# fukangl/SMG-multimodal-grasping

Hardware: AMD Instinct MI355X
Metric: affordance fwd+bwd passes/sec (16-rot 224^2 RGB-D) (higher is better)
Workload: dtype f32; 1 GPU; 16 rot x 224^2 (S=640): fwd + Huber + bwd + Adam per GPU per step; reinforcement_net style 0; 17 trunk passes; fp32; leg=headline, rotations=16, input_size=640, parallelism=dp1

## Files before the change

### smg-multimodal-grasping_amd/csrc/backward.hip

```cpp
#include "engine.h"

int do_backward(smg_engine* e, const smg_net* net, const float* dq, hipStream_t st, int phases, bool elem_head) {
    if (!e->have_fwd) return fail(-22, "smg_backward without a preceding smg_forward");
    if (!net->grads) return fail(-22, "net.grads is NULL");
    if (phases == 2 && !e->bw_phase0_done)
        return fail(-22, "smg_backward_phase(1) must follow smg_backward_phase(0) of the same forward");
    if ((phases & 1) && e->bw_phase0_done)
        return fail(-22, "smg_backward / smg_backward_phase(0) while the second half of a two-phase backward is still due (run phase 1 or a new forward)");
    const Layout& L = *e->L;
    const TrunkRef& T = L.trunk[e->f_trunk];
    const HeadRef& Hd = L.head[e->f_head];
    const int NS = e->f_streams, NP = e->f_pairs;
    const float* P = net->params;
    float* Gr = net->grads;
    const Plane p4 = e->p_blk[3];
    const bool ph_a = phases & 1, ph_b = phases & 2;
    if (ph_a) {
        for (int r = 0; r < kStatRep; ++r) HIP_OK(hipMemsetAsync(e->bstat + (size_t)r * kStatRepStride, 0, 2 * e->bstat_span * sizeof(double), st));
    }
    const bool split16 = e->prec == 0 && kSplitOp == 3;
    if (ph_a && split16) HIP_OK(hipMemsetAsync(e->gamax, 0, (size_t)e->gamax_words * sizeof(unsigned), st));
    const hipStream_t s2 = (e->prof || e->serialize) ? st : e->side;
    auto fork = [&](hipEvent_t ev) -> int {
        HIP_OK(hipEventRecord(ev, st));
        HIP_OK(hipStreamWaitEvent(s2, ev, 0));
        return 0;
    };
    const bool gs_materialised = split16 || NS > 4;
    auto gs_on_side = [&](const Plane& pl) { return split16 && !e->generic3x3 && pl.HW <= 1600 && NS <= 4; };
    auto fused_gsrc = [&](int b, const DenseLayerRef& d) {
        return grad_src(e, e->G[b], kBlockCtot[b], e->X[b], kBlockCtot[b], e->st_X[b], d.cin, nullptr);
    };
    auto launch_gs_apply = [&](int b, int i, hipStream_t cs, float* GSb, const GradSrc& fused) {
        const Plane pl = e->p_blk[b];
        BnBwdApplyArgs a{};
        a.src = fused; a.src.xtab = stat_table(e, e->sx_tab[b], e->max_streams, kBlockCtot[b], T.layers[b][i].cin);
        a.pl = pl; a.C = kGrowth;
        a.out = GSb; a.ldo = kGrowth; a.amax = split16 ? gamax_of(e, b, i, 0) : nullptr;
        PREC_DISPATCH(e, launch_kernel(e, bn_bwd_apply_kernel<PREC>, dim3((pl.HWp + bn_apply_rows(PREC) - 1) / bn_apply_rows(PREC), NS), dim3(256), 0, cs,
                                       K_OTHER, 0, ESZ(e) * NS * pl.HW * 3 * kGrowth, false, a));
    };

    auto norm1_src = [&](int b, int i, int c0) {
        const DenseLayerRef& d = T.layers[b][i];
        return act_src(e, e->X[b], kBlockCtot[b], e->st_X[b], c0, P + d.n1.w, P + d.n1.b, stat_table(e, e->sx_tab[b], e->max_streams, kBlockCtot[b]), asc_n1(e, b, i));
    };
    auto norm2_src = [&](int b, int i) {
        const DenseLayerRef& d = T.layers[b][i];
        return act_src(e, el(e, e->Bt, e->bt_off[b][i]), kBottleneck, e->st_Bt[b][i], 0, P + d.n2.w, P + d.n2.b,
                       !e->generic3x3 ? stat_table(e, e->sb_tab[b][i], e->max_streams, kBottleneck) : StatTab{}, asc_n2(e, b, i));
    };

    PartialTiles tiles(e->part_floats, NS, e->deterministic);

    if (ph_a) {
    {
        ValueBwdArgs a;
        a.h1 = head_norm1_src(e, Hd, P); a.p4 = p4; a.w2p = e->packed_f + e->pk_head1;
        a.dq = dq; a.out_ch = e->head_out; a.OH = e->OH; a.OW = e->OW; a.dh1 = e->DH1;
        a.st = stat_sink_bwd(e, e->st_H1, 0); a.aff = affine_sink(Gr, Hd.n1); a.dw2 = Gr + Hd.c1.w;
        const bool dense = !elem_head && (e->head_bwd == 2 || (e->head_bwd == 0 && e->f_dense_dq));
        if (!dense) {
// ... 190 lines not shown
                a.wu = e->packed_u + e->pk_hd[b][i];
                const double flops = 2.0 * NS * pl.HW * 9 * kBottleneck * kGrowth;
                const double bytes = ESZ(e) * NS * pl.HW * (kGrowth + 2 * kBottleneck);
                if (halo_tile(pl, NS) == 16) {
                    a.tiles_x = (pl.W + 15) / 16; a.cg_per_wg = kBottleneck / 32;
                    if (pl.H % 16 || pl.W % 16) {
                        PREC_DISPATCH(e, launch_kernel(e, conv3x3_halo_dgrad_kernel<16, PREC, true>, dim3(((pl.H + 15) / 16) * a.tiles_x, NS), dim3(256),
                                                       HaloDgradSGeo<16, PREC>::smem_bytes(kBottleneck), st, K_D3, flops, bytes, true, a));
                    } else {
                        PREC_DISPATCH(e, launch_kernel(e, conv3x3_halo_dgrad_kernel<16, PREC>, dim3((pl.H / 16) * a.tiles_x, NS), dim3(256),
                                                       HaloDgradSGeo<16, PREC>::smem_bytes(kBottleneck), st, K_D3, flops, bytes, true, a));
                    }
                } else {
                    a.tiles_x = (pl.W + 7) / 8; a.cg_per_wg = 1;
                    PREC_DISPATCH(e, launch_kernel(e, conv3x3_halo_dgrad_kernel<8, PREC>, dim3(((pl.H + 7) / 8) * a.tiles_x, NS, kBottleneck / 64), dim3(256),
                                                   HaloDgradSGeo<8, PREC>::smem_bytes(kBottleneck), st, K_D3, flops, bytes, true, a));
                }
            } else {
                auto run = [&](auto tag) {
                    using Cfg = decltype(tag);
                    BwdDataP<Cfg, true, E_STORE, false> p{};
                    p.gs = grad_done(GSb, kGrowth); p.pa = pl; p.KA = kGrowth;
                    p.wp = e->packed_u + e->pk_g3d[b][i]; p.K8tot = 9 * kGrowth / 8; p.ldn = kBottleneck; p.wcol0 = 0; p.N = kBottleneck;
                    p.m = n2; p.pm = pl;
                    p.dst = split16 ? e->DY2 : D2b; p.ldd = kBottleneck; p.dcoff = 0;
                    p.st = n2st; p.aff = affine_sink(Gr, d.n2);
                    launch_gemm(e, st, p, dim3(NS * pl.HWp / Cfg::BM, kBottleneck / Cfg::BN), K_D3, 2.0 * NS * pl.HW * 9 * kBottleneck * kGrowth,
                                ESZ(e) * NS * pl.HW * (kGrowth + 2 * kBottleneck));
                };
                if (pl.HWp % 128 == 0) run(CfgP128x128{}); else run(CfgP64x128{});
            }
            const GradSrc dy2 = grad_src(e, split16 ? e->DY2 : D2b, kBottleneck, bt, kBottleneck, e->st_Bt[b][i], 0, P + d.n2.w,
                                         !e->generic3x3 ? stat_table(e, e->sb_tab[b][i], e->max_streams, kBottleneck) : StatTab{});
            if (split16) {
                BnBwdApplySplitArgs a{};
                a.src = dy2; a.pl = pl; a.out = reinterpret_cast<u32x4*>(D2b); a.binv = lb.D2S;
                if (!e->generic3x3) a.aff = affine_sink(Gr, d.n2);
                launch_kernel(e, bn_bwd_apply_split_kernel, dim3(pl.HWp / kScaleBlock, NS), dim3(256), 0, st, K_OTHER, 0, 4.0 * NS * pl.HW * 3 * kBottleneck, false, a);
            } else {
                if (e->dbg_stop == b * 100 + i) {
                    if (int rc = dbg_snapshot(e->dbg_dy2, e->dbg_dy2_floats, e->dbg_dy2_n, D2b, (int64_t)NS * pl.HWp * kBottleneck)) return rc;
                }
                BnBwdApplyArgs a{};
                a.src = dy2; a.pl = pl; a.C = kBottleneck; a.out = D2b; a.ldo = kBottleneck;
                if (!e->generic3x3) a.aff = affine_sink(Gr, d.n2);
                PREC_DISPATCH(e, launch_kernel(e, bn_bwd_apply_kernel<PREC>, dim3((pl.HWp + bn_apply_rows(PREC) - 1) / bn_apply_rows(PREC), NS), dim3(256), 0, st,
                                               K_OTHER, 0, ESZ(e) * NS * pl.HW * 3 * kBottleneck, false, a));
            }
            if (fork(e->ev_d2[lb.ring % kRing])) return -5;
            if (int rc = issue_wgrads(b, i)) return rc;
            HIP_OK(hipEventRecord(e->ev_side[lb.ring % kRing], s2));
            if (e->dbg_stop == b * 100 + i) {
                if (int rc = dbg_snapshot(e->dbg_gsnap, e->dbg_gsnap_floats, e->dbg_gsnap_n, e->G[b], (int64_t)NS * pl.HWp * Ct)) return rc;
            }
            const int L = (int)T.layers[b].size();
            const int g_lo = i - ((L - 1 - i) % kGroup == kGroup - 1 ? 0 : std::min(i, kGroup - 1 - (L - 1 - i) % kGroup));
            const int cs = T.layers[b][g_lo].cin;
            if (d.cin > cs) {
                auto run = [&](auto tag, auto ptag) {
                    using Cfg = MC<decltype(tag), decltype(ptag)::value>;
                    BwdDataP<Cfg, false, E_ACCUM, false, decltype(ptag)::value> p{};
                    p.gs = grad_done(D2b, kBottleneck); p.pa = pl; p.KA = kBottleneck; p.binv = lb.D2S;
                    p.wp = e->packed_u + e->pk_d1[b][i]; p.K8tot = kBottleneck / 8; p.ldn = d.cin; p.wcol0 = cs; p.N = d.cin - cs;
                    p.m = norm1_src(b, i, cs); p.pm = pl;
                    p.dst = e->G[b]; p.ldd = Ct; p.dcoff = cs;
                    p.st = stat_sink_bwd(e, e->st_X[b], cs); p.aff = affine_sink_scr(e, e->db_off[b][i], d.cin, cs);
                    launch_gemm(e, st, p, dim3(NS * pl.HWp / Cfg::BM, (p.N + Cfg::BN - 1) / Cfg::BN), K_D1, 2.0 * NS * pl.HW * p.N * kBottleneck,
                                ESZ(e) * NS * pl.HW * (kBottleneck + 3.0 * p.N));
                };
                PREC_DISPATCH(e, if (pl.HWp % 128 == 0) run(CfgP128x64{}, PTAG); else run(CfgP64x64{}, PTAG));
            }
            if (i == g_lo) {
                auto run = [&](auto tag, auto ptag) {
                    using Cfg = MC<decltype(tag), decltype(ptag)::value>;
                    BwdDataGroupP<Cfg, decltype(ptag)::value> p{};
                    const int g_hi = L - 1 - ((L - 1 - g_lo) / kGroup) * kGroup;
                    p.nseg = g_hi - g_lo + 1;
                    for (int k = 0; k < p.nseg; ++k) {
                        const DenseLayerRef& dk = T.layers[b][g_lo + k];
                        const LayerBuf lk = buf_of(b, g_lo + k);
                        p.seg[k].g = lk.D2; p.seg[k].wp = e->packed_u + e->pk_d1[b][g_lo + k]; p.seg[k].ldn = dk.cin; p.seg[k].binv = lk.D2S;
                        p.seg[k].gamma = P + dk.n1.w; p.seg[k].beta = P + dk.n1.b;
                        p.seg[k].aff = affine_sink_scr(e, e->db_off[b][g_lo + k], dk.cin, 0);
                    }
                    p.ldg = kBottleneck; p.pa = pl; p.KA = kBottleneck; p.N = cs;
                    p.m = act_src(e, e->X[b], Ct, e->st_X[b], 0, nullptr, nullptr, stat_table(e, e->sx_tab[b], e->max_streams, Ct));
                    p.dst = e->G[b]; p.ldd = Ct;
                    p.st = stat_sink_bwd(e, e->st_X[b], 0);
                    launch_gemm(e, st, p, dim3(NS * pl.HWp / Cfg::BM, (cs + Cfg::BN - 1) / Cfg::BN), K_D1, 2.0 * NS * pl.HW * cs * kBottleneck * p.nseg,
                                ESZ(e) * NS * pl.HW * ((double)p.nseg * kBottleneck + 3.0 * cs));
                };
// ... 125 lines not shown
```

### smg-multimodal-grasping_amd/csrc/elem.cuh

```cuda
#pragma once
#include "gemm.cuh"

namespace smg {

struct PrepArgs {
    const float* images_nchw;
    const double* heightmaps;
    int hm, pad, S;
    double mean, stdv;
    const int* stream_image;
    const float* stream_affine;
    const int* stream_rotated;
    float* img4;
    float* img1;
    int HWp;
    const double* masks;
    const int* stream_mask_a;
    const int* stream_mask_b;
};

__device__ __forceinline__ float lin_coord(int i, int S, float step) {
    return (i < S / 2) ? fmaf(step, (float)i, -1.f) : fmaf(-step, (float)(S - 1 - i), 1.f);
}

// ... 1089 lines not shown
            if constexpr (E == 4) {
                const float4 o = affine2(gv[k], xv[k], prm + 4 * cs, a.C);
                stq<GT>(a.out, pix * a.ldo + 4 * cs, o);
                vmax = fmaxf(fmaxf(vmax, fmaxf(fabsf(o.x), fabsf(o.y))), fmaxf(fabsf(o.z), fabsf(o.w)));
            } else {
                const u32x4 u = pack_unit<1>(affine2(slot_quad<GT>(gv[k], 0), slot_quad<XT>(xv[k], 0), prm + 8 * cs, a.C),
                                             affine2(slot_quad<GT>(gv[k], 1), slot_quad<XT>(xv[k], 1), prm + 8 * cs + 4, a.C));
                *reinterpret_cast<u32x4*>(static_cast<char*>(a.out) + (int64_t)GT::size * (pix * a.ldo + 8 * cs)) = u;
            }
        }
    }
    if constexpr (E == 4) {
        if (a.amax) {
#pragma unroll
            for (int o = 32; o > 0; o >>= 1) vmax = fmaxf(vmax, __shfl_xor(vmax, o));
            __syncthreads();
            if ((t & 63) == 0) prm[t >> 6] = vmax;
            __syncthreads();
            if (t == 0) {
                vmax = fmaxf(fmaxf(prm[0], prm[1]), fmaxf(prm[2], prm[3]));
                if (vmax > 0.f) atomicMax(a.amax + (int64_t)n * kAmaxRep + (blockIdx.x % kAmaxRep), __float_as_uint(vmax));
            }
        }
    }
}

struct BnBwdApplySplitArgs {
    GradSrc src;
    Plane pl;
    u32x4* out;
    float* binv;
    AffineSink aff;
};
static __global__ __launch_bounds__(256) void bn_bwd_apply_split_kernel(const BnBwdApplySplitArgs a) {
    constexpr int C = 8 * kD2K8;
    __shared__ float prm[4 * C];
    __shared__ float red[4];
    const int n = blockIdx.y, t = threadIdx.x;
    const int cs = t >> 3, rr = t & 7;
    const int r0 = blockIdx.x * kScaleBlock + rr;
    float4 gv[8], xv[8];
#pragma unroll
    for (int k = 0; k < 8; ++k) {
        const int r = r0 + 8 * k;
        const int64_t pix = (int64_t)n * a.pl.HWp + (r < a.pl.HW ? r : 0);
        gv[k] = ld4(static_cast<const float*>(a.src.g) + pix * C + 4 * cs);
        xv[k] = ld4(static_cast<const float*>(a.src.x) + pix * C + 4 * cs);
    }
    if (t < C) {
        const double inv = 1.0 / (double)a.pl.HW;
        float mean, invstd;
        const GradSrc& g = a.src;
        tab_or_moments(g.xtab, n, t, g.xsum, g.xsq, (int64_t)n * g.sstride + t, inv, g.eps, mean, invstd);
        const double s1 = stat_get(g.s1, (int64_t)n * g.sstride + t), s2 = stat_get(g.s2, (int64_t)n * g.sstride + t);
        prm[t] = g.gamma[t] * invstd;
        prm[C + t] = (float)(s1 * inv);
        prm[2 * C + t] = mean;
        prm[3 * C + t] = invstd * (float)(s2 * inv);
        if (a.aff.dbeta && blockIdx.x == 0) affine_sink_add2(a.aff, t, (float)s1, (float)s2);
    }
    __syncthreads();
    float vmax = 0.f;
#pragma unroll
    for (int k = 0; k < 8; ++k) {
        const float4 o = r0 + 8 * k < a.pl.HW ? affine2(gv[k], xv[k], prm + 4 * cs, C) : zero4();
        gv[k] = o;
        vmax = fmaxf(fmaxf(vmax, fmaxf(fabsf(o.x), fabsf(o.y))), fmaxf(fabsf(o.z), fabsf(o.w)));
    }
#pragma unroll
    for (int o = 32; o > 0; o >>= 1) vmax = fmaxf(vmax, __shfl_xor(vmax, o));
    if ((t & 63) == 0) red[t >> 6] = vmax;
    __syncthreads();
    vmax = fmaxf(fmaxf(red[0], red[1]), fmaxf(red[2], red[3]));
    ActScale sc{1.f, 1.f};
    if (vmax > 0.f) sc = scale_of_max(__float_as_uint(vmax));
    if (t == 0) a.binv[(int64_t)n * (a.pl.HWp / kScaleBlock) + blockIdx.x] = sc.inv;
    char* ob = reinterpret_cast<char*>(a.out + d2_stream_units(n, a.pl.HWp));
#pragma unroll
    for (int k = 0; k < 8; ++k) {
        const Split4 s = split4<3>(mul4(gv[k], sc.s));
        const int64_t at = ((int64_t)(cs >> 1) * a.pl.HWp + r0 + 8 * k) * 16 + (cs & 1) * 8;
        *reinterpret_cast<uint2*>(ob + at) = s.p[0];
        *reinterpret_cast<uint2*>(ob + at + (int64_t)kD2K8 * a.pl.HWp * 16) = s.p[1];
    }
}

struct DbSegD { int64_t grad_off; int scr_off; int n; };
static __global__ void db_flush_kernel(const DbSegD* segs, float* scr, int rep_stride, int reps, float* grads,
                                       const double* stem1, const double* stem2, int ns, float* dbeta0, float* dgamma0) {
    if (blockIdx.y == gridDim.y - 1) {
        if (blockIdx.x == 0 && threadIdx.x < 128 && stem1) {
            const int q = threadIdx.x >> 6, c = threadIdx.x & 63;
            double v = 0.0;
            for (int n = 0; n < ns; ++n) v += stat_get(q ? stem2 : stem1, (int64_t)n * 64 + c);
            (q ? dgamma0 : dbeta0)[c] += (float)v;
        }
        return;
    }
    const DbSegD sg = segs[blockIdx.y];
    for (int k = blockIdx.x * blockDim.x + threadIdx.x; k < sg.n; k += gridDim.x * blockDim.x) {
        float v = 0.f;
        for (int r = 0; r < reps; ++r) {
            float* q = scr + (int64_t)r * rep_stride + sg.scr_off + k;
            v += *q;
            *q = 0.f;
        }
        grads[sg.grad_off + k] += v;
    }
}

template <int PREC>
static __global__ void zero_uncovered_kernel(void* G, int ld, Plane p, int Hc, int Wc, int C) {
    using GT = grd_t<PREC>;
    const int n = blockIdx.y;
    const int64_t total = (int64_t)p.HW * (C / 4);
    for (int64_t i = blockIdx.x * (int64_t)blockDim.x + threadIdx.x; i < total; i += (int64_t)gridDim.x * blockDim.x) {
        const int pix = (int)(i / (C / 4)), cq = (int)(i - (int64_t)pix * (C / 4));
// ... 219 lines not shown
```

### smg-multimodal-grasping_amd/csrc/engine.h

```cpp
#pragma once
#include <hip/hip_runtime.h>

#include <algorithm>
#include <cmath>
#include <cstdio>
#include <cstdlib>
#include <cstring>
#include <string>
#include <type_traits>
#include <vector>

#include "../../include/smg_hip.h"
#include "elem.cuh"
#include "scene.cuh"
#include "gemm.cuh"
#include "halo.cuh"
#include "ws.cuh"
#include "wsw.cuh"
#include "plan.h"

using namespace smg;

int smg_fail(int code, const std::string& msg);
static inline int fail(int code, const std::string& msg) { return smg_fail(code, msg); }
#define HIP_OK(expr)                                                                              \
    do {                                                                                          \
        hipError_t _e = (expr);                                                                   \
        if (_e != hipSuccess)                                                                     \
            return fail(-5, std::string(#expr) + ": " + hipGetErrorString(_e));                   \
    } while (0)

static const Layout& layout_for(int head_out) {
    static Layout L1 = build_layout(1);
    static Layout L3 = build_layout(3);
    return head_out == 3 ? L3 : L1;
}

using CfgP128x128 = GemmCfg<128, 128, 16, 2, 2, 1, true>;
using CfgP128x32 = GemmCfg<128, 32, 32, 4, 1, 1, true>;
using CfgP128x64 = GemmCfg<128, 64, 16, 2, 2, 1, true>;
using CfgP64x64 = GemmCfg<64, 64, 32, 2, 2, 1, true>;
using CfgP32x64 = GemmCfg<32, 64, 32, 1, 2, 2, true>;
using CfgP64x128 = GemmCfg<64, 128, 16, 2, 2, 1, true>;
using CfgP64x32 = GemmCfg<64, 32, 64, 2, 1, 2, true>;
using CfgW32x128 = GemmCfg<32, 128, 32, 1, 4, 1, false>;
using CfgW128x64 = GemmCfg<128, 64, 16, 2, 2, 1, false>;
using CfgW128x128 = GemmCfg<128, 128, 16, 2, 2, 1, false>;
using CfgW64x64 = GemmCfg<64, 64, 16, 2, 2, 1, false>;
using CfgW64x256 = GemmCfg<64, 256, 16, 2, 2, 1, false>;

template <class C, int PREC, int MUL = 2>
// ... 34 lines not shown
    StatArr st_stem, st_X[4], st_F, st_H1; std::vector<StatArr> st_Bt[4];
    u32x4* packed_u = nullptr; int64_t packed_units = 0;
    float* packed_f = nullptr; int64_t packed_floats = 0;
    PackDesc* d_pack = nullptr; std::vector<PackDesc> h_pack[3]; std::vector<PackDesc> h_pack_head[3];
    int pack_stride = 0, bnupd_stride = 0, n_bnupd = 0;
    int64_t pk_conv0 = 0, pk_conv0_1 = 0, pk_head0 = 0, pk_hd0 = 0, pk_head1 = 0;
    std::vector<int64_t> pk_c1[4], pk_d1[4], pk_g3f[4], pk_g3d[4], pk_hf[4], pk_hd[4]; int64_t pk_t[3] = {}, pk_td[3] = {};
    int max_pack = 0;
    float* asc = nullptr; ActScaleDesc* d_asc = nullptr; int n_asc = 0;
    unsigned* gamax = nullptr; int64_t gamax_words = 0;
    float* stab = nullptr; int64_t stab_floats = 0;
    int64_t sx_tab[4] = {}, sb_tab[4][24] = {}, sf_tab = 0;
    BnUpdDesc* d_bnupd = nullptr;
    bool have_fwd = false; int f_trunk = 0, f_head = 0, f_streams = 0, f_pairs = 0;
    bool bw_phase0_done = false;
    bool f_dense_dq = false;
    int head_bwd = 0;
    bool f_stem1 = false;
    int* d_stream_image = nullptr; int* d_stream_rot = nullptr; int* d_pair_a = nullptr; int* d_pair_b = nullptr;
    int* d_seq_t = nullptr; int* d_seq_h = nullptr; int* d_user_ptr = nullptr; int* d_user_pair = nullptr; int* d_user_slot = nullptr;
    float* d_affine = nullptr;
    float* scene_val = nullptr; int* scene_idx = nullptr; int scene_tiles = 0;
    double* scene_lpart = nullptr;
    double* scene_gpart = nullptr; int* scene_cnt = nullptr;
    int* d_stage = nullptr; int* h_stage[2] = {}; hipEvent_t ev_stage[2] = {}; int stage_ints = 0, stage_turn = 0;
    int so_image = 0, so_rot = 0, so_pa = 0, so_pb = 0, so_seq_t = 0, so_seq_h = 0, so_uptr = 0, so_upair = 0, so_uslot = 0, so_aff = 0, so_ma = 0, so_mb = 0, so_adam = 0;
    bool capturing = false; int* h_stage_g = nullptr; hipEvent_t ev_graph = nullptr, ev_gin = nullptr; hipStream_t gstream = nullptr; struct StepGraph* step_graph = nullptr;
    int64_t workspace_bytes = 0;
    int n_cu = 256;
    int prec = 0;
    bool serialize = false;
    bool deterministic = false;
    bool generic3x3 = false, generic_c1 = false, generic_w1 = false, stem_plane_tail = false;
    float* stemv = nullptr; float* mom_part = nullptr; double* mom = nullptr; int mom_groups = 0;
    int dbg_stop = -1;
    float* dbg_gsnap = nullptr; int64_t dbg_gsnap_floats = 0; int64_t dbg_gsnap_n = 0;
    float* dbg_dy2 = nullptr; int64_t dbg_dy2_floats = 0; int64_t dbg_dy2_n = 0;
    int dbg_snap_prec = -1;
    bool prof = false; std::vector<ProfRec> recs; std::vector<hipEvent_t> ev_pool;
    double prof_ms[5][K_COUNT] = {}; int64_t prof_n[5][K_COUNT] = {}; double prof_flops[5][K_COUNT] = {}; double prof_bytes[5][K_COUNT] = {}; int prof_stage = -1;
    int launch_rc = 0;
};

constexpr int kMomTilesPerWg = 8;
static inline int stem_mom_tiles_x(const Plane& ps) { return (ps.W + kMomT - 1) / kMomT; }
static inline int stem_mom_tiles(const Plane& ps) { return stem_mom_tiles_x(ps) * ((ps.H + kMomT - 1) / kMomT); }
static inline int stem_mom_groups(const Plane& ps) { return (stem_mom_tiles(ps) + kMomTilesPerWg - 1) / kMomTilesPerWg; }

static Plane make_plane(int H, int W) {
    Plane p; p.H = H; p.W = W; p.HW = H * W;
    const int g = p.HW >= 8192 ? 128 : 64;
    p.HWp = (p.HW + g - 1) / g * g;
    return p;
}

template <class T>
static int dev_alloc(smg_engine* e, T** out, int64_t count) {
    void* p = nullptr;
    hipError_t err = hipMalloc(&p, (size_t)count * sizeof(T));
    if (err != hipSuccess) return fail(-12, std::string("hipMalloc ") + std::to_string(count * sizeof(T)) + " B: " + hipGetErrorString(err));
    e->workspace_bytes += count * (int64_t)sizeof(T);
    *out = (T*)p;
    return 0;
}
#define ALLOC(ptr, count) do { int _r = dev_alloc(e, &(ptr), (count)); if (_r) return _r; } while (0)

// ... 227 lines not shown
```

### smg-multimodal-grasping_amd/csrc/engine.hip

```cpp
#include "engine.h"

static thread_local std::string g_err;
int smg_fail(int code, const std::string& msg) { g_err = msg; return code; }

static int zero_typed_buffers(smg_engine* e) {
    const int NS = e->max_streams;
    for (int b = 0; b < 4; ++b) {
        const size_t n = (size_t)NS * e->p_blk[b].HWp * kBlockCtot[b] * sizeof(float);
        HIP_OK(hipMemset(e->X[b], 0, n));
        HIP_OK(hipMemset(e->G[b], 0, n));
    }
    HIP_OK(hipMemset(e->Bt, 0, (size_t)e->bt_floats * sizeof(float)));
    for (int k = 0; k < kRing; ++k) {
        HIP_OK(hipMemset(e->D2[k], 0, (size_t)NS * e->p_blk[0].HWp * kBottleneck * sizeof(float)));
        HIP_OK(hipMemset(e->GS[k], 0, (size_t)NS * e->p_blk[0].HWp * kGrowth * sizeof(float)));
    }
    HIP_OK(hipMemset(e->DY2, 0, (size_t)NS * e->p_blk[0].HWp * kBottleneck * sizeof(float)));
    HIP_OK(hipDeviceSynchronize());
    return 0;
}

static int engine_build(smg_engine* e) {
    const Layout& L = *e->L;
    const int NS = e->max_streams, NP = e->max_pairs;
    const int S = e->S;
    const int H1 = (S - 1) / 2 + 1, H2 = (H1 - 1) / 2 + 1;
    e->p_img = make_plane(S, S);
    e->p_stem = make_plane(H1, H1);
    int h = H2;
    for (int b = 0; b < 4; ++b) { e->p_blk[b] = make_plane(h, h); h /= 2; }
    e->OH = e->OW = e->p_blk[3].H - kHeadKernel + 1;
    if (e->OH < 1) return fail(-22, "input_size too small for the 20x20 value head");

    if (getenv("SMG_SERIALIZE")) e->serialize = true;
    const int cross = getenv("SMG_CROSSCHECK") ? atoi(getenv("SMG_CROSSCHECK")) : 0;
    e->generic3x3 = cross & 1; e->generic_c1 = cross & 2; e->generic_w1 = cross & 4; e->stem_plane_tail = cross & 8;

    ALLOC(e->img4, (int64_t)NS * e->p_img.HWp * 4);
    ALLOC(e->stem, (int64_t)NS * e->p_stem.HWp * 64);
    ALLOC(e->DY0, (int64_t)NS * e->p_stem.HWp * 64);
    ALLOC(e->argmax, (int64_t)NS * e->p_blk[0].HWp * 64);
    e->stemv = e->DY0;
    e->mom_groups = stem_mom_groups(e->p_stem);
    ALLOC(e->mom_part, (int64_t)NS * e->mom_groups * kMomVals);
    ALLOC(e->mom, (int64_t)NS * kMomOut);
    int64_t bt_total = 0;
    for (int b = 0; b < 4; ++b) {
        ALLOC(e->X[b], (int64_t)NS * e->p_blk[b].HWp * kBlockCtot[b]);
        ALLOC(e->G[b], (int64_t)NS * e->p_blk[b].HWp * kBlockCtot[b]);
        for (int i = 0; i < kBlockLayers[b]; ++i) {
            e->bt_off[b].push_back(bt_total);
            bt_total += (int64_t)NS * e->p_blk[b].HWp * kBottleneck;
        }
    }
    ALLOC(e->Bt, bt_total);
    for (int k = 0; k < kRing; ++k) {
        ALLOC(e->D2[k], (int64_t)NS * e->p_blk[0].HWp * kBottleneck);
        ALLOC(e->GS[k], (int64_t)NS * e->p_blk[0].HWp * kGrowth);
        ALLOC(e->D2S[k], (int64_t)NS * (e->p_blk[0].HWp / kScaleBlock));
        HIP_OK(hipEventCreateWithFlags(&e->ev_gs[k], hipEventDisableTiming));
        HIP_OK(hipEventCreateWithFlags(&e->ev_d2[k], hipEventDisableTiming));
        HIP_OK(hipEventCreateWithFlags(&e->ev_side[k], hipEventDisableTiming));
    }
    ALLOC(e->DY2, (int64_t)NS * e->p_blk[0].HWp * kBottleneck);
    e->bt_floats = bt_total;
    if (int rc = zero_typed_buffers(e)) return rc;
    e->scene_tiles = (int)(((int64_t)(S / 2) * (S / 2) + kSceneTile - 1) / kSceneTile);
    ALLOC(e->scene_val, (int64_t)kSceneMaps * e->scene_tiles);
    ALLOC(e->scene_idx, (int64_t)kSceneMaps * e->scene_tiles);
// ... 791 lines not shown
    if (rc == 0) {
        HIP_OK(hipEventRecord(e->ev_graph, st));
        HIP_OK(hipStreamWaitEvent(caller, e->ev_graph, 0));
    }
    return rc;
}

int smg_engine_set_precision(smg_engine* e, int precision) {
    if (!e) return fail(-22, "engine is NULL");
    if (precision < 0 || precision > 2) return fail(-22, "precision must be 0 (fp32 storage, fp32-class split products), 1 (bf16 storage) or 2 (fp16 activations, bf16 gradients)");
    if (precision && e->generic3x3) return fail(-22, "SMG_CROSSCHECK=1 (the generic implicit-GEMM 3x3 path) exists in the fp32-class mode only");
    if (precision != e->prec) {
        HIP_OK(hipSetDevice(e->device));
        HIP_OK(hipDeviceSynchronize());
        if (int rc = zero_typed_buffers(e)) return rc;
    }
    e->prec = precision;
    step_graph_drop(e);
    e->have_fwd = false;
    e->bw_phase0_done = false;
    return 0;
}

int smg_engine_set_option(smg_engine* e, const char* name, int value) {
    if (!e || !name) return fail(-22, "NULL argument");
    const std::string s(name);
    if (s == "deterministic") { e->deterministic = value != 0; return 0; }
    if (s == "head_bwd") {
        if (value < 0 || value > 2) return fail(-22, "head_bwd must be 0 (follow the mark of smg_loss_map / smg_loss_map_ce), 1 (per-element form) or 2 (dense form)");
        e->head_bwd = value; return 0;
    }
    if (s == "serialize") { e->serialize = value != 0; return 0; }
    if (s == "debug_stop") { e->dbg_stop = value; return 0; }
    return fail(-22, "unknown engine option '" + s + "'");
}

int smg_heightmap(const double* depth_img_dev, int h, int w, const double* intrinsics3x3, const double* cam_pose4x4,
                  const double* inv_homography3x3, int out_w, int out_h, double* out_dev, void* stream) {
    if (!depth_img_dev || !intrinsics3x3 || !cam_pose4x4 || !inv_homography3x3 || !out_dev || h < 1 || w < 1 || out_w < 1 || out_h < 1)
        return fail(-22, "bad heightmap arguments");
    hipPointerAttribute_t attr;
    HIP_OK(hipPointerGetAttributes(&attr, depth_img_dev));
    HIP_OK(hipSetDevice(attr.device));
    HeightmapArgs a;
    a.depth = depth_img_dev; a.h = h; a.w = w;
    a.fx = intrinsics3x3[0]; a.fy = intrinsics3x3[4]; a.cx = intrinsics3x3[2]; a.cy = intrinsics3x3[5];
    a.r20 = cam_pose4x4[8]; a.r21 = cam_pose4x4[9]; a.r22 = cam_pose4x4[10]; a.t2 = cam_pose4x4[11];
    for (int i = 0; i < 9; ++i) a.mi[i] = inv_homography3x3[i];
    a.out = out_dev; a.ow = out_w; a.oh = out_h;
    hipLaunchKernelGGL(heightmap_warp_kernel, dim3((out_w + 255) / 256, out_h), dim3(256), 0, (hipStream_t)stream, a);
    HIP_OK(hipGetLastError());
    return 0;
}

int smg_argmax(const float* values_dev, int n, int* idx_out_dev, float* val_out_dev, void* stream) {
    if (!values_dev || !idx_out_dev || !val_out_dev || n < 1) return fail(-22, "bad argmax arguments");
    hipPointerAttribute_t attr;
    HIP_OK(hipPointerGetAttributes(&attr, values_dev));
    HIP_OK(hipSetDevice(attr.device));
    hipLaunchKernelGGL(argmax_kernel, dim3(1), dim3(256), 0, (hipStream_t)stream, values_dev, n, idx_out_dev, val_out_dev);
    HIP_OK(hipGetLastError());
    return 0;
}

int smg_adam_step(float* params, const float* grads, float* m, float* v, int64_t offset, int64_t count, int step, float lr,
                  float beta1, float beta2, float eps, void* stream) {
// ... 71 lines not shown
    } else if (s == "dy2") {
        src = e->dbg_dy2; n = e->dbg_dy2_n;
        if (!src) return fail(-22, "dy2: no debug_stop backward has run in a 16-bit mode");
        if (e->dbg_snap_prec != e->prec) return fail(-22, "dy2: taken in another precision mode");
    } else if (s.size() == 5 && s.substr(0, 4) == "fs_x") {
        const int b = s[4] - '1';
        if (b < 0 || b > 3) return fail(-22, "bad fs_x name");
        const int64_t nd = (int64_t)NS * kBlockCtot[b];
        n = 4 * nd;
        if (!host_out) return n;
        if (cap < n) return fail(-22, "fs_x: buffer too small");
        HIP_OK(hipSetDevice(e->device));
        HIP_OK(hipStreamSynchronize((hipStream_t)stream));
        HIP_OK(hipMemcpy(host_out, fsum(e, e->st_X[b]), (size_t)nd * sizeof(double), hipMemcpyDeviceToHost));
        HIP_OK(hipMemcpy(host_out + 2 * nd, fsq(e, e->st_X[b]), (size_t)nd * sizeof(double), hipMemcpyDeviceToHost));
        return n;
    } else if (s.size() == 5 && s.substr(0, 4) == "bs_x") {
        const int b = s[4] - '1';
        if (b < 0 || b > 3) return fail(-22, "bad bs_x name");
        const int64_t nd = (int64_t)NS * kBlockCtot[b];
        n = 4 * nd;
        if (!host_out) return n;
        if (cap < n) return fail(-22, "bs_x: buffer too small");
        HIP_OK(hipSetDevice(e->device));
        HIP_OK(hipStreamSynchronize((hipStream_t)stream));
        std::vector<double> tot((size_t)2 * nd, 0.0), rep((size_t)nd);
        for (int q = 0; q < 2; ++q)
            for (int r = 0; r < kStatRep; ++r) {
                HIP_OK(hipMemcpy(rep.data(), (q ? b2(e, e->st_X[b]) : b1(e, e->st_X[b])) + (int64_t)r * kStatRepStride, (size_t)nd * sizeof(double), hipMemcpyDeviceToHost));
                for (int64_t k = 0; k < nd; ++k) tot[(size_t)(q * nd + k)] += rep[(size_t)k];
            }
        std::memcpy(host_out, tot.data(), tot.size() * sizeof(double));
        return n;
    } else if (s.size() >= 5 && (s.substr(0, 3) == "gs_" || s.substr(0, 3) == "d2_")) {
        int b = 0, i = 0;
        if (std::sscanf(name + 3, "%d_%d", &b, &i) != 2 || b < 1 || b > 4 || i < 1 || i > kBlockLayers[b - 1]) return fail(-22, "bad ring buffer name");
        const int slot = ring_pos(b - 1, i - 1) % kRing;
        const Plane& pl = e->p_blk[b - 1];
        const bool gs = s[0] == 'g';
        const int64_t per_stream = (int64_t)pl.HWp * (gs ? kGrowth : kBottleneck);
        n = (int64_t)NS * per_stream;
        if (!host_out) return n;
        const int ns_out = (int)std::min<int64_t>(NS, cap / per_stream);
        n = ns_out * per_stream;
        HIP_OK(hipSetDevice(e->device));
        HIP_OK(hipStreamSynchronize((hipStream_t)stream));
        if (e->prec != 0) {
            std::vector<unsigned short> raw((size_t)n);
            HIP_OK(hipMemcpy(raw.data(), gs ? e->GS[slot] : e->D2[slot], raw.size() * sizeof(unsigned short), hipMemcpyDeviceToHost));
            widen16(raw.data(), n, false, host_out);
            return n;
        }
        if (gs || kSplitOp != 3) {
            HIP_OK(hipMemcpy(host_out, gs ? e->GS[slot] : e->D2[slot], n * sizeof(float), hipMemcpyDeviceToHost));
            return n;
        }
        std::vector<unsigned short> u((size_t)ns_out * per_stream * 2);
        std::vector<float> inv((size_t)NS * (pl.HWp / kScaleBlock));
        HIP_OK(hipMemcpy(u.data(), e->D2[slot], u.size() * sizeof(unsigned short), hipMemcpyDeviceToHost));
        HIP_OK(hipMemcpy(inv.data(), e->D2S[slot], inv.size() * sizeof(float), hipMemcpyDeviceToHost));
        auto h2f = [](unsigned h) -> double {
            const int ex = (h >> 10) & 31, man = h & 1023;
            const double v = ex == 0 ? std::ldexp((double)man, -24) : (ex == 31 ? (man ? NAN : INFINITY) : std::ldexp((double)(man | 1024), ex - 25));
            return (h & 0x8000u) ? -v : v;
        };
        for (int sn = 0; sn < ns_out; ++sn)
// ... 81 lines not shown
```

Measured before the change: 63.71 passes/s.

## Fuse norm2 backward apply with per-layer 1x1 data-gradient GEMM

Adds a kernel that performs the split-precision norm2 backward apply and, keeping the resulting packed gradient tile in shared memory, immediately runs the 1x1 conv data-gradient MFMA product for the layer's new channels, accumulating into the block gradient and its BN statistics. This removes a separate GEMM launch and the global re-read of the D2 buffer per dense layer. The fused kernel assumes at most 96 output columns and multiples of 32, and trades GEMM tiling flexibility and occupancy for fewer passes over memory. An engine option and environment variable allow turning it off.

```diff
diff --git a/smg-multimodal-grasping_amd/csrc/apply_dgrad.cuh b/smg-multimodal-grasping_amd/csrc/apply_dgrad.cuh
--- /dev/null
+++ b/smg-multimodal-grasping_amd/csrc/apply_dgrad.cuh
@@ -0,0 +1,130 @@
+#pragma once
+#include "elem.cuh"
+#include "gemm.cuh"
+
+namespace smg {
+
+struct ApplyDgradArgs {
+    BnBwdApplySplitArgs ap;
+    const u32x4* wp; int ldn; int wcol0; int N;
+    ActSrc m;
+    float* dst; int ldd; int dcoff;
+    StatSink st; AffineSink aff;
+};
+
+constexpr int kApplyDgradMaxN = 96;
+
+static __global__ __launch_bounds__(256, 2) void apply_dgrad_kernel(const ApplyDgradArgs a) {
+    __shared__ __attribute__((aligned(16))) char tile[kD2TileBytes];
+    __shared__ float red[4];
+    static_assert(kD2TileBytes >= (int)sizeof(float) * 4 * 8 * kD2K8 && kD2TileBytes >= (int)sizeof(float) * 4 * kApplyDgradMaxN, "overlays");
+    const int n = blockIdx.y, t = threadIdx.x, lane = t & 63, wave = t >> 6, l31 = lane & 31, half = lane >> 5;
+    const int rt = wave & 1, ct0 = wave >> 1, NT = a.N >> 5;
+    const int pbase = blockIdx.x * kScaleBlock;
+    const Plane pl = a.ap.pl;
+
+    ApplySplitRows R;
+    apply_split_fetch(a.ap, R);
+
+    bool has[2];
+    u32x4 bw[2][2][8];
+    float xv[2][16], gold[2][16];
+    float p_sc[2], p_sh[2], p_mean[2], p_inv[2], p_gam[2];
+    const u32x4* wcol = a.wp + a.wcol0 + l31;
+    auto load_b = [&](int q) {
+#pragma unroll
+        for (int pc = 0; pc < 2; ++pc)
+#pragma unroll
+            for (int s = 0; s < 8; ++s) bw[q][pc][s] = wcol[(int64_t)((pc * kD2K8 + 2 * s + half) * a.ldn + (ct0 + 2 * q) * 32)];
+    };
+    const int64_t srow = (int64_t)n * pl.HWp;
+#pragma unroll
+    for (int q = 0; q < 2; ++q) {
+        has[q] = ct0 + 2 * q < NT;
+        if (!has[q]) continue;
+        const int cj = (ct0 + 2 * q) * 32 + l31;
+        if (q == 0) load_b(0);
+        const ActCoef f = act_src_coef(a.m, n, cj, 1.0 / (double)pl.HW);
+        p_sc[q] = f.gamma * f.invstd; p_sh[q] = f.beta; p_mean[q] = f.mean; p_inv[q] = f.invstd; p_gam[q] = f.gamma;
+#pragma unroll
+        for (int r = 0; r < 16; ++r) {
+            const int row = pbase + rt * 32 + (r & 3) + 8 * (r >> 2) + 4 * half;
+            const int64_t pix = srow + (row < pl.HW ? row : 0);
+            xv[q][r] = static_cast<const float*>(a.m.x)[pix * a.m.ldx + cj];
+            gold[q][r] = a.dst[pix * a.ldd + a.dcoff + cj];
+        }
+    }
+
+    const ActScale sc = apply_split_finish<true>(a.ap, R, reinterpret_cast<float*>(tile), red, tile);
+    if (pbase >= pl.HW) return;
+    if (has[1]) load_b(1);
+    __syncthreads();
+
+    f32x16 acc[2];
+#pragma unroll
+    for (int q = 0; q < 2; ++q)
+#pragma unroll
+        for (int r = 0; r < 16; ++r) acc[q][r] = 0.f;
+    const char* arow = tile + (half * kD2TileLdu + rt * 32 + l31) * 16;
+#pragma unroll
+    for (int q = 0; q < 2; ++q) {
+        if (!has[q]) continue;
+#pragma unroll
+        for (int s = 0; s < 8; ++s) {
+            const u32x4 ah = *reinterpret_cast<const u32x4*>(arow + (2 * s) * kD2TileLdu * 16);
+            const u32x4 al = *reinterpret_cast<const u32x4*>(arow + (kD2K8 + 2 * s) * kD2TileLdu * 16);
+            acc[q] = mfma_f16(ah, bw[q][1][s], acc[q]);
+            acc[q] = mfma_f16(al, bw[q][0][s], acc[q]);
+            acc[q] = mfma_f16(ah, bw[q][0][s], acc[q]);
+        }
+    }
+
+    const float gi = sc.inv * pack_inv_scale(a.wp);
+    float v[2][2];
+#pragma unroll
+    for (int q = 0; q < 2; ++q) {
+        v[0][q] = v[1][q] = 0.f;
+        if (!has[q]) continue;
+        const int cj = (ct0 + 2 * q) * 32 + l31;
+#pragma unroll
+        for (int r = 0; r < 16; ++r) {
+            const int row = pbase + rt * 32 + (r & 3) + 8 * (r >> 2) + 4 * half;
+            const bool rok = row < pl.HW;
+            const float av = acc[q][r] * gi;
+            const float xr = xv[q][r];
+            const float dy = (rok && bn1(xr, p_mean[q], p_sc[q], p_sh[q]) > 0.f) ? av : 0.f;
+            if (rok) a.dst[(srow + row) * a.ldd + a.dcoff + cj] = gold[q][r] + p_gam[q] * dy;
+            v[0][q] += dy;
+            v[1][q] += dy * ((xr - p_mean[q]) * p_inv[q]);
+        }
+    }
+    float* cred = reinterpret_cast<float*>(tile);
+#pragma unroll
+    for (int k = 0; k < 2; ++k)
+#pragma unroll
+        for (int q = 0; q < 2; ++q) v[k][q] += __shfl_xor(v[k][q], 32);
+    __syncthreads();
+    if (half == 0) {
+#pragma unroll
+        for (int k = 0; k < 2; ++k)
+#pragma unroll
+            for (int q = 0; q < 2; ++q)
+                if (has[q]) cred[(k * 2 + rt) * kApplyDgradMaxN + (ct0 + 2 * q) * 32 + l31] = v[k][q];
+    }
+    __syncthreads();
+    if (t < a.N) {
+        float tot[2];
+#pragma unroll
+        for (int k = 0; k < 2; ++k) {
+            float s = 0.f;
+            s += cred[(k * 2 + 0) * kApplyDgradMaxN + t];
+            s += cred[(k * 2 + 1) * kApplyDgradMaxN + t];
+            tot[k] = s;
+        }
+        const float wgt = a.m.gamma[t];
+        stat_sink_add2<S_BWD>(a.st, n, t, (double)(wgt * tot[0]), (double)(wgt * tot[1]));
+        affine_sink_add2(a.aff, t, tot[0], tot[1]);
+    }
+}
+
+}
diff --git a/smg-multimodal-grasping_amd/csrc/backward.hip b/smg-multimodal-grasping_amd/csrc/backward.hip
--- a/smg-multimodal-grasping_amd/csrc/backward.hip
+++ b/smg-multimodal-grasping_amd/csrc/backward.hip
@@ -28,6 +28,7 @@
     };
     const bool gs_materialised = split16 || NS > 4;
     auto gs_on_side = [&](const Plane& pl) { return split16 && !e->generic3x3 && pl.HW <= 1600 && NS <= 4; };
+    auto apply_dgrad_on = [&](const Plane&) { return e->apply_dgrad != 0; };
     auto fused_gsrc = [&](int b, const DenseLayerRef& d) {
         return grad_src(e, e->G[b], kBlockCtot[b], e->X[b], kBlockCtot[b], e->st_X[b], d.cin, nullptr);
     };
@@ -284,10 +285,27 @@
             }
             const GradSrc dy2 = grad_src(e, split16 ? e->DY2 : D2b, kBottleneck, bt, kBottleneck, e->st_Bt[b][i], 0, P + d.n2.w,
                                          !e->generic3x3 ? stat_table(e, e->sb_tab[b][i], e->max_streams, kBottleneck) : StatTab{});
+            const int L = (int)T.layers[b].size();
+            const int g_lo = i - ((L - 1 - i) % kGroup == kGroup - 1 ? 0 : std::min(i, kGroup - 1 - (L - 1 - i) % kGroup));
+            const int cs = T.layers[b][g_lo].cin;
+            const bool apply_forms_d1 = split16 && !e->generic3x3 && d.cin > cs && apply_dgrad_on(pl);
+            if (e->dbg_stop == b * 100 + i) {
+                if (int rc = dbg_snapshot(e->dbg_gsnap, e->dbg_gsnap_floats, e->dbg_gsnap_n, e->G[b], (int64_t)NS * pl.HWp * Ct)) return rc;
+            }
             if (split16) {
                 BnBwdApplySplitArgs a{};
                 a.src = dy2; a.pl = pl; a.out = reinterpret_cast<u32x4*>(D2b); a.binv = lb.D2S;
                 if (!e->generic3x3) a.aff = affine_sink(Gr, d.n2);
+                if (apply_forms_d1) {
+                    ApplyDgradArgs f{};
+                    f.ap = a;
+                    f.wp = e->packed_u + e->pk_d1[b][i]; f.ldn = d.cin; f.wcol0 = cs; f.N = d.cin - cs;
+                    f.m = norm1_src(b, i, cs);
+                    f.dst = e->G[b]; f.ldd = Ct; f.dcoff = cs;
+                    f.st = stat_sink_bwd(e, e->st_X[b], cs); f.aff = affine_sink_scr(e, e->db_off[b][i], d.cin, cs);
+                    launch_kernel(e, apply_dgrad_kernel, dim3(pl.HWp / kScaleBlock, NS), dim3(256), 0, st, K_D1, 2.0 * NS * pl.HW * f.N * kBottleneck,
+                                  4.0 * NS * pl.HW * (3.0 * kBottleneck + 3.0 * f.N), false, f);
+                } else
                 launch_kernel(e, bn_bwd_apply_split_kernel, dim3(pl.HWp / kScaleBlock, NS), dim3(256), 0, st, K_OTHER, 0, 4.0 * NS * pl.HW * 3 * kBottleneck, false, a);
             } else {
                 if (e->dbg_stop == b * 100 + i) {
@@ -302,13 +320,7 @@
             if (fork(e->ev_d2[lb.ring % kRing])) return -5;
             if (int rc = issue_wgrads(b, i)) return rc;
             HIP_OK(hipEventRecord(e->ev_side[lb.ring % kRing], s2));
-            if (e->dbg_stop == b * 100 + i) {
-                if (int rc = dbg_snapshot(e->dbg_gsnap, e->dbg_gsnap_floats, e->dbg_gsnap_n, e->G[b], (int64_t)NS * pl.HWp * Ct)) return rc;
-            }
-            const int L = (int)T.layers[b].size();
-            const int g_lo = i - ((L - 1 - i) % kGroup == kGroup - 1 ? 0 : std::min(i, kGroup - 1 - (L - 1 - i) % kGroup));
-            const int cs = T.layers[b][g_lo].cin;
-            if (d.cin > cs) {
+            if (d.cin > cs && !apply_forms_d1) {
                 auto run = [&](auto tag, auto ptag) {
                     using Cfg = MC<decltype(tag), decltype(ptag)::value>;
                     BwdDataP<Cfg, false, E_ACCUM, false, decltype(ptag)::value> p{};
diff --git a/smg-multimodal-grasping_amd/csrc/elem.cuh b/smg-multimodal-grasping_amd/csrc/elem.cuh
--- a/smg-multimodal-grasping_amd/csrc/elem.cuh
+++ b/smg-multimodal-grasping_amd/csrc/elem.cuh
@@ -1145,21 +1145,30 @@
     float* binv;
     AffineSink aff;
 };
-static __global__ __launch_bounds__(256) void bn_bwd_apply_split_kernel(const BnBwdApplySplitArgs a) {
+struct ApplySplitRows { float4 gv[8], xv[8]; };
+constexpr int kD2TileLdu = kScaleBlock + 8;
+constexpr int kD2TileBytes = 2 * kD2K8 * kD2TileLdu * 16;
+__device__ __forceinline__ void apply_split_fetch(const BnBwdApplySplitArgs& a, ApplySplitRows& R) {
     constexpr int C = 8 * kD2K8;
-    __shared__ float prm[4 * C];
-    __shared__ float red[4];
     const int n = blockIdx.y, t = threadIdx.x;
     const int cs = t >> 3, rr = t & 7;
     const int r0 = blockIdx.x * kScaleBlock + rr;
-    float4 gv[8], xv[8];
 #pragma unroll
     for (int k = 0; k < 8; ++k) {
         const int r = r0 + 8 * k;
         const int64_t pix = (int64_t)n * a.pl.HWp + (r < a.pl.HW ? r : 0);
-        gv[k] = ld4(static_cast<const float*>(a.src.g) + pix * C + 4 * cs);
-        xv[k] = ld4(static_cast<const float*>(a.src.x) + pix * C + 4 * cs);
-    }
+        R.gv[k] = ld4(static_cast<const float*>(a.src.g) + pix * C + 4 * cs);
+        R.xv[k] = ld4(static_cast<const float*>(a.src.x) + pix * C + 4 * cs);
+    }
+}
+template <bool TILE>
+__device__ __forceinline__ ActScale apply_split_finish(const BnBwdApplySplitArgs& a, ApplySplitRows& R, float* prm, float* red, char* tile) {
+    constexpr int C = 8 * kD2K8;
+    float4 (&gv)[8] = R.gv;
+    float4 (&xv)[8] = R.xv;
+    const int n = blockIdx.y, t = threadIdx.x;
+    const int cs = t >> 3, rr = t & 7;
+    const int r0 = blockIdx.x * kScaleBlock + rr;
     if (t < C) {
         const double inv = 1.0 / (double)a.pl.HW;
         float mean, invstd;
@@ -1195,7 +1204,20 @@
         const int64_t at = ((int64_t)(cs >> 1) * a.pl.HWp + r0 + 8 * k) * 16 + (cs & 1) * 8;
         *reinterpret_cast<uint2*>(ob + at) = s.p[0];
         *reinterpret_cast<uint2*>(ob + at + (int64_t)kD2K8 * a.pl.HWp * 16) = s.p[1];
-    }
+        if constexpr (TILE) {
+            char* tp = tile + ((cs >> 1) * kD2TileLdu + rr + 8 * k) * 16 + (cs & 1) * 8;
+            *reinterpret_cast<uint2*>(tp) = s.p[0];
+            *reinterpret_cast<uint2*>(tp + kD2K8 * kD2TileLdu * 16) = s.p[1];
+        }
+    }
+    return sc;
+}
+static __global__ __launch_bounds__(256) void bn_bwd_apply_split_kernel(const BnBwdApplySplitArgs a) {
+    __shared__ float prm[4 * 8 * kD2K8];
+    __shared__ float red[4];
+    ApplySplitRows R;
+    apply_split_fetch(a, R);
+    apply_split_finish<false>(a, R, prm, red, nullptr);
 }
 
 struct DbSegD { int64_t grad_off; int scr_off; int n; };
diff --git a/smg-multimodal-grasping_amd/csrc/engine.h b/smg-multimodal-grasping_amd/csrc/engine.h
--- a/smg-multimodal-grasping_amd/csrc/engine.h
+++ b/smg-multimodal-grasping_amd/csrc/engine.h
@@ -17,6 +17,7 @@
 #include "halo.cuh"
 #include "ws.cuh"
 #include "wsw.cuh"
+#include "apply_dgrad.cuh"
 #include "plan.h"
 
 using namespace smg;
@@ -117,6 +118,7 @@
     bool serialize = false;
     bool deterministic = false;
     bool generic3x3 = false, generic_c1 = false, generic_w1 = false, stem_plane_tail = false;
+    int apply_dgrad = -1;
     float* stemv = nullptr; float* mom_part = nullptr; double* mom = nullptr; int mom_groups = 0;
     int dbg_stop = -1;
     float* dbg_gsnap = nullptr; int64_t dbg_gsnap_floats = 0; int64_t dbg_gsnap_n = 0;
diff --git a/smg-multimodal-grasping_amd/csrc/engine.hip b/smg-multimodal-grasping_amd/csrc/engine.hip
--- a/smg-multimodal-grasping_amd/csrc/engine.hip
+++ b/smg-multimodal-grasping_amd/csrc/engine.hip
@@ -35,6 +35,7 @@
     if (getenv("SMG_SERIALIZE")) e->serialize = true;
     const int cross = getenv("SMG_CROSSCHECK") ? atoi(getenv("SMG_CROSSCHECK")) : 0;
     e->generic3x3 = cross & 1; e->generic_c1 = cross & 2; e->generic_w1 = cross & 4; e->stem_plane_tail = cross & 8;
+    if (const char* v = getenv("SMG_APPLY_DGRAD")) e->apply_dgrad = std::max(-1, std::min(1, atoi(v)));
 
     ALLOC(e->img4, (int64_t)NS * e->p_img.HWp * 4);
     ALLOC(e->stem, (int64_t)NS * e->p_stem.HWp * 64);
@@ -892,6 +893,10 @@
     }
     if (s == "serialize") { e->serialize = value != 0; return 0; }
     if (s == "debug_stop") { e->dbg_stop = value; return 0; }
+    if (s == "apply_dgrad") {
+        if (value < -1 || value > 1) return fail(-22, "apply_dgrad must be -1 (the walk's rule), 0 (norm2 apply and per-layer 1x1 data gradient as two kernels) or 1 (one kernel wherever a layer has the product)");
+        e->apply_dgrad = value; step_graph_drop(e); return 0;
+    }
     return fail(-22, "unknown engine option '" + s + "'");
 }
 
@@ -1029,6 +1034,14 @@
             }
         std::memcpy(host_out, tot.data(), tot.size() * sizeof(double));
         return n;
+    } else if (s.size() >= 6 && (s.substr(0, 4) == "d2u_" || s.substr(0, 4) == "d2s_")) {
+        int b = 0, i = 0;
+        if (e->prec != 0 || kSplitOp != 3) return fail(-22, "d2u / d2s: the unit form exists in precision mode 0 only");
+        if (std::sscanf(name + 4, "%d_%d", &b, &i) != 2 || b < 1 || b > 4 || i < 1 || i > kBlockLayers[b - 1]) return fail(-22, "bad ring buffer name");
+        const int slot = ring_pos(b - 1, i - 1) % kRing;
+        const Plane& pl = e->p_blk[b - 1];
+        if (s[2] == 'u') { src = e->D2[slot]; n = (int64_t)NS * pl.HWp * kBottleneck; }
+        else { src = e->D2S[slot]; n = (int64_t)NS * (pl.HWp / kScaleBlock); }
     } else if (s.size() >= 5 && (s.substr(0, 3) == "gs_" || s.substr(0, 3) == "d2_")) {
         int b = 0, i = 0;
         if (std::sscanf(name + 3, "%d_%d", &b, &i) != 2 || b < 1 || b > 4 || i < 1 || i > kBlockLayers[b - 1]) return fail(-22, "bad ring buffer name");
```

After: 63.69 passes/s. About the same (-0.0%).
